# edlanglois/relearn

Hardware: AMD Instinct MI355X
Metric: env-steps/sec (whole node), 64k-env CartPole TRPO (higher is better)
Workload: dtype f32; 1 GPU; CartPole(VisibleStepLimit 500) MLP-TRPO, 65536 envs total, T=128, policy 5-128-2, critic 5-128-1, CG 10, <=15 backtracks, 80 Adam critic steps per period; n_envs_total=65536, n_envs_per_gpu=65536, horizon=128, hidden=128, critic_steps=80, update_chains=policy and critic chains side by side on two streams, pipeline=none, parallelism=env-sharded x1 + no collective (one rank)

## Files before the change

### include/relearn_hip.h

```cpp
#ifndef RELEARN_HIP_H
#define RELEARN_HIP_H

#include <stddef.h>
#include <stdint.h>

#ifdef __cplusplus
extern "C" {
#endif

#define RL_ABI_VERSION 6

typedef enum {
  RL_OK = 0,
  RL_ERR_INVALID_ARGUMENT = 1,
  RL_ERR_HIP = 2,
  RL_ERR_NO_DEVICE = 3,
  RL_ERR_BUILD_AGENT = 4,
  RL_ERR_BUILD_ENV = 5,
  RL_ERR_BUFFER_FULL = 6,
  RL_ERR_PACKING = 7,
  RL_ERR_COMM = 8,
  RL_ERR_OPT_NAN = 9,
  RL_ERR_UNSUPPORTED = 10
} rl_status;
// ... 117 lines not shown
enum { RL_CELL_GRU = 0, RL_CELL_LSTM = 1 };
int32_t rl_rnn_mlp_create(rl_engine *engine, int32_t cell, uint32_t in_dim, uint32_t hidden_size, uint32_t num_layers,
                          uint32_t mlp_hidden, uint32_t out_dim, rl_mlp **out);
int32_t rl_rnn_mlp_create_config(rl_engine *engine, int32_t cell, uint32_t in_dim, uint32_t hidden_size,
                                 uint32_t num_layers, int32_t bias, uint32_t mlp_hidden, uint32_t out_dim, rl_mlp **out);

typedef enum {
  RL_TRAJ_OBS = 0,
  RL_TRAJ_ACTION = 1,
  RL_TRAJ_REWARD = 2,
  RL_TRAJ_FLAG = 3,
  RL_TRAJ_TERM_OBS = 4,
  RL_TRAJ_VALUES = 5,
  RL_TRAJ_ADVANTAGES = 6,
  RL_TRAJ_RETURNS = 7,
  RL_TRAJ_TARGETS = 8
} rl_traj_field;

int32_t rl_traj_create(rl_engine *engine, uint64_t n_lanes, uint64_t horizon, uint32_t obs_dim, rl_traj **out);
int32_t rl_traj_destroy(rl_traj *traj);
int32_t rl_traj_field_bytes(const rl_traj *traj, int32_t field, uint64_t *bytes);
int32_t rl_traj_read(rl_traj *traj, int32_t field, void *host, uint64_t bytes);
int32_t rl_traj_write(rl_traj *traj, int32_t field, const void *host, uint64_t bytes);

int32_t rl_rollout(rl_env *env, const rl_mlp *policy, rl_traj *traj);

int32_t rl_gae(rl_traj *traj, const rl_mlp *critic, float gamma, float lambda);
int32_t rl_seq_forward(rl_mlp *module, rl_traj *traj, float *out, float *succ_out);

typedef struct {
  uint64_t iterations;
// ... 169 lines not shown
```

### relearn_amd/__init__.py

```python
import atexit
import ctypes as C
import math
import os
import subprocess
import sys
import weakref

import numpy as np

_HERE = os.path.dirname(os.path.abspath(__file__))
LIB_PATH = os.environ.get("RELEARN_LIB", os.path.join(_HERE, "librelearn_hip.so"))
CSRC = os.path.join(_HERE, "csrc")

OK = 0
ERR_INVALID_ARGUMENT, ERR_HIP, ERR_NO_DEVICE, ERR_BUILD_AGENT, ERR_BUILD_ENV = 1, 2, 3, 4, 5
ERR_BUFFER_FULL, ERR_PACKING, ERR_COMM, ERR_OPT_NAN, ERR_UNSUPPORTED = 6, 7, 8, 9, 10
SUCC_CONTINUE, SUCC_TERMINATE, SUCC_INTERRUPT = 0, 1, 2
OPT_OK, OPT_LOSS_NOT_IMPROVING, OPT_CONSTRAINT_VIOLATED, OPT_NAN_LOSS, OPT_NAN_CONSTRAINT = range(5)
ENV_CARTPOLE, ENV_CHAIN, ENV_MEMORY, ENV_BANDIT = 0, 1, 2, 3
LIMIT_NONE, LIMIT_LATENT, LIMIT_VISIBLE = 0, 1, 2
(TRAJ_OBS, TRAJ_ACTION, TRAJ_REWARD, TRAJ_FLAG, TRAJ_TERM_OBS, TRAJ_VALUES, TRAJ_ADVANTAGES,
 TRAJ_RETURNS, TRAJ_TARGETS) = range(9)
VALUE_TARGET_REWARD_TO_GO, VALUE_TARGET_ONE_STEP_TD = 0, 1
KERNEL_CLASSES = ["env_step", "rollout", "values", "gae", "policy_pass", "backward", "reduce", "small",
                  "critic_fwd", "allreduce", "critic_fused", "policy_fused", "policy_fvp"]

ABI_SYMBOLS = [
    "rl_abi_version", "rl_debug_stream_words", "rl_device_count", "rl_engine_create", "rl_engine_destroy", "rl_engine_sync",
    "rl_last_error", "rl_engine_info", "rl_engine_set_kernel_variant", "rl_timer_begin", "rl_timer_end", "rl_profile_enable", "rl_profile_read",
    "rl_comm_available", "rl_comm_library_paths", "rl_comm_unique_id", "rl_comm_init", "rl_comm_destroy", "rl_comm_init_host",
    "rl_comm_ipc_handle", "rl_comm_init_ipc", "rl_comm_selftest",
    "rl_cartpole_params_default", "rl_env_create", "rl_env_destroy", "rl_env_dims", "rl_env_reset",
    "rl_env_observe", "rl_env_step", "rl_env_upload_actions", "rl_env_step_resident", "rl_env_get_state",
    "rl_env_set_state",
    "rl_mlp_create", "rl_mlp_create_layers", "rl_mlp_create_config", "rl_mlp_destroy", "rl_mlp_num_params", "rl_mlp_init", "rl_mlp_init_with", "rl_params_get", "rl_params_set",
    "rl_mlp_forward", "rl_gru_mlp_create", "rl_lstm_mlp_create", "rl_rnn_mlp_create", "rl_rnn_mlp_create_config", "rl_rnn_mlp_init_with", "rl_seq_forward",
    "rl_traj_create", "rl_traj_destroy", "rl_traj_field_bytes", "rl_traj_read", "rl_traj_write",
# ... 521 lines not shown
    def forward(self, rows):
        rows, rp = _ptr(rows, np.float32)
        out = np.zeros((rows.shape[0], self.out_dim), dtype=np.float32)
        _check(lib().rl_mlp_forward(self.h, rp, C.c_uint64(rows.shape[0]), out.ctypes.data_as(C.c_void_p)),
               self.eng.h)
        return out


GruMlp.close = Mlp.close
GruMlp.init = Mlp.init
GruMlp.get_params = Mlp.get_params
GruMlp.set_params = Mlp.set_params

_TRAJ_DTYPES = {TRAJ_OBS: np.float32, TRAJ_ACTION: np.uint8, TRAJ_REWARD: np.float32, TRAJ_FLAG: np.uint8,
                TRAJ_TERM_OBS: np.float32, TRAJ_VALUES: np.float32, TRAJ_ADVANTAGES: np.float32,
                TRAJ_RETURNS: np.float32, TRAJ_TARGETS: np.float32}


class Trajectory(_Handle):
    def __init__(self, engine, n_lanes, horizon, obs_dim):
        self.eng = engine
        self.h = C.c_void_p()
        _check(lib().rl_traj_create(engine.h, C.c_uint64(n_lanes), C.c_uint64(horizon), C.c_uint32(obs_dim),
                                    C.byref(self.h)), engine.h)
        _register(self)
        self.n, self.T, self.D = n_lanes, horizon, obs_dim

    def close(self):
        if self.h:
            lib().rl_traj_destroy(self.h)
            self.h = C.c_void_p()

    def shape(self, field):
        n, T, D = self.n, self.T, self.D
        return {TRAJ_OBS: (D, T + 1, n), TRAJ_ACTION: (T, n), TRAJ_REWARD: (T, n), TRAJ_FLAG: (T, n),
                TRAJ_TERM_OBS: (D, T, n), TRAJ_VALUES: (T + 1, n), TRAJ_ADVANTAGES: (T, n),
                TRAJ_RETURNS: (T, n), TRAJ_TARGETS: (T, n)}[field]

    def read(self, field):
        out = np.zeros(self.shape(field), dtype=_TRAJ_DTYPES[field])
        _check(lib().rl_traj_read(self.h, C.c_int32(field), out.ctypes.data_as(C.c_void_p),
                                  C.c_uint64(out.nbytes)), self.eng.h)
        return out

    def write(self, field, arr):
        arr, ap = _ptr(arr, _TRAJ_DTYPES[field])
        assert arr.shape == self.shape(field), (arr.shape, self.shape(field))
        _check(lib().rl_traj_write(self.h, C.c_int32(field), ap, C.c_uint64(arr.nbytes)), self.eng.h)

    def read_all(self):
        return dict(obs=self.read(TRAJ_OBS), action=self.read(TRAJ_ACTION), reward=self.read(TRAJ_REWARD),
                    flag=self.read(TRAJ_FLAG), term_obs=self.read(TRAJ_TERM_OBS))
# ... 427 lines not shown
```

### relearn_amd/csrc/abi.hip

```cpp
#include <dlfcn.h>

#include <atomic>
#include <condition_variable>
#include <map>
#include <mutex>

#include "abi_internal.hpp"

thread_local std::string g_last_error_no_engine;

ProfScope::ProfScope(rl_engine *eng, int c) : e(eng), cls(c) {
  if (!e->profiling) return;
  auto get = [&]() {
    hipEvent_t ev;
    if (!e->prof_event_pool.empty()) {
      ev = e->prof_event_pool.back();
      e->prof_event_pool.pop_back();
    } else if (hipEventCreate(&ev) != hipSuccess) {
      ev = nullptr;
    }
    return ev;
  };
  a = get();
  b = get();
// ... 1273 lines not shown
  uint64_t n = t->d.n, T = t->d.T, D = t->d.D;
  switch (field) {
    case RL_TRAJ_OBS: *ptr = t->d.obs; *bytes = D * (T + 1) * n * 4; break;
    case RL_TRAJ_ACTION: *ptr = t->d.action; *bytes = T * n; break;
    case RL_TRAJ_REWARD: *ptr = t->d.reward; *bytes = T * n * 4; break;
    case RL_TRAJ_FLAG: *ptr = t->d.flag; *bytes = T * n; break;
    case RL_TRAJ_TERM_OBS: *ptr = t->d.term_obs; *bytes = D * T * n * 4; break;
    case RL_TRAJ_VALUES: *ptr = t->d.values; *bytes = (T + 1) * n * 4; break;
    case RL_TRAJ_ADVANTAGES: *ptr = t->d.adv; *bytes = T * n * 4; break;
    case RL_TRAJ_RETURNS: *ptr = t->d.rtg; *bytes = T * n * 4; break;
    case RL_TRAJ_TARGETS:
      RL_REQUIRE(t->last_targets != nullptr, "no value targets yet: they are written by rl_values_opt_update");
      *ptr = const_cast<float *>(t->last_targets);
      *bytes = T * n * 4;
      break;
    default: throw RlError(RL_ERR_INVALID_ARGUMENT, "unknown trajectory field");
  }
}

void traj_plan(rl_traj *t, uint64_t B) {
  rl_engine *e = t->eng;
  t->B = B;
  uint64_t chunk = (B + 1023) / 1024;
  chunk = ((chunk + 7) / 8) * 8;
  if (chunk < 64) chunk = 64;
  t->bwd_chunk = (uint32_t)chunk;
  t->nbA = (uint32_t)((B + chunk - 1) / chunk);
  uint64_t nbB = (B + 255) / 256;
  if (nbB > 2048) nbB = 2048;
  t->nbB = (uint32_t)nbB;
// ... 31 lines not shown
  t->d.tgt = t->d.rtg;
  t->d.range = dalloc<uint32_t>(RL_RANGE_ALLOC_WORDS);
  RL_HIP_CHECK(hipMemsetAsync(t->d.range, 0, RL_RANGE_ALLOC_WORDS * sizeof(uint32_t), e->stream));
  {
    void *hp = nullptr;
    RL_HIP_CHECK(hipHostMalloc(&hp, 64, hipHostMallocMapped));
    static_cast<volatile uint32_t *>(hp)[RL_GUARD_POLICY] = 0u;
    static_cast<volatile uint32_t *>(hp)[RL_GUARD_CRITIC] = 0u;
    void *dp = nullptr;
    RL_HIP_CHECK(hipHostGetDevicePointer(&dp, hp, 0));
    t->h_range_err = static_cast<uint32_t *>(hp);
    t->d.range_err = static_cast<uint32_t *>(dp);
  }
  t->lp0 = dalloc<float>(2 * n * T);
  t->dz = dalloc<float>(2 * n * T);
  t->Pmax = 128 * 5 + 128 + 2 * 128 + 2;
  traj_plan(t.get(), n * T);
  uint32_t rows = t->nbA;
  if (t->nbV2 > rows) rows = t->nbV2;
  if (t->nbC > rows) rows = t->nbC;
  uint32_t rowsB = t->nbB > rows ? t->nbB : rows;
  if (resizable) {
    uint32_t cap = 8u * (uint32_t)e->prop.multiProcessorCount;
    if (cap < 2048) cap = 2048;
    rows = rowsB = cap;
  }
  t->slabA = dalloc<double>((size_t)rows * t->Pmax);
  t->slabB = dalloc<double>((size_t)rowsB * 4);
  t->cap_slabA = (uint64_t)rows * t->Pmax;
  t->cap_slabB = (uint64_t)rowsB * 4;
// ... 21 lines not shown
    RL_REQUIRE(e && out, "NULL argument");
    *out = nullptr;
    *out = traj_alloc(e, n_lanes, horizon, obs_dim, false);
  });
}

static void seq_free(rl_traj *t);

int32_t rl_traj_destroy(rl_traj *t) {
  if (!t) return RL_OK;
  (void)hipSetDevice(t->eng->device);
  (void)hipStreamSynchronize(t->eng->main_stream);
  (void)hipStreamSynchronize(t->eng->aux_stream);
  if (t->eng->pending.traj == t) t->eng->pending.active = false;
  void *ptrs[] = {t->d.obs, t->d.action, t->d.reward, t->d.flag, t->d.term_obs, t->d.values, t->d.adv, t->d.rtg,
                  t->lp0, t->dz, t->slabA, t->slabB, t->vec, t->cg_x, t->cg_r, t->cg_p, t->prev_params, t->descent,
                  t->losses, t->trpo, t->td, t->aux_slabA, t->aux_slabB, t->aux_vec, t->d.range};
  for (void *p : ptrs) dfree(p);
  if (t->h_range_err) (void)hipHostFree(t->h_range_err);
  seq_free(t);
  gen_free(t);
  rl_engine *eng = t->eng;
  delete t;
  engine_release_child(eng);
  return RL_OK;
}

int32_t rl_traj_field_bytes(const rl_traj *t, int32_t field, uint64_t *bytes) {
  return guarded(t ? t->eng : nullptr, [&] {
    RL_REQUIRE(t && bytes, "NULL argument");
    void *p;
// ... 5 lines not shown
  return guarded(t ? t->eng : nullptr, [&] {
    RL_REQUIRE(t && host, "NULL argument");
    void *p;
    uint64_t need;
    traj_field(t, field, &p, &need);
    RL_REQUIRE(bytes == need, "byte count mismatch for trajectory field");
    d2h(t->eng, host, p, bytes);
  });
}

int32_t rl_traj_write(rl_traj *t, int32_t field, const void *host, uint64_t bytes) {
  return guarded(t ? t->eng : nullptr, [&] {
    RL_REQUIRE(t && host, "NULL argument");
    void *p;
    uint64_t need;
    traj_field(t, field, &p, &need);
    RL_REQUIRE(bytes == need, "byte count mismatch for trajectory field");
    h2d(t->eng, p, host, bytes);
    if (field == RL_TRAJ_OBS) t->range_valid = t->range_reset = false;
    t->rtg_scan_valid = false;
  });
}

void traj_ensure_pvec(rl_traj *t, uint64_t P) {
  if (t->Pmax >= P) return;
  for (float **p : {&t->vec, &t->cg_x, &t->cg_r, &t->cg_p, &t->prev_params, &t->descent}) {
    dfree(*p);
    *p = nullptr;
  }
  t->Pmax = (uint32_t)P;
// ... 117 lines not shown
```

### relearn_amd/csrc/abi_update.hip

```cpp
#include "abi_internal.hpp"

extern "C" {

static void seq_gradient_to_flat_order(const rl_mlp *mod, rl_traj *traj) {
  if (mod->exec == nullptr) return;
  launch_seq_unpad(mod, traj->vec, mod->x_tmp);
  RL_HIP_CHECK(hipMemcpyAsync(traj->vec, mod->x_tmp, mod->P * sizeof(float), hipMemcpyDeviceToDevice, traj->eng->stream));
}

static float *seq_record(rl_traj *traj, const rl_mlp *mod) {
  return mod->lane_kernels() ? traj->seq.stack.rec : traj->seq.act;
}

static void seq_policy_pass(rl_mlp *policy, rl_traj *traj, int mode, bool backward, float lo, float hi) {
  SeqScope sc(traj, policy);
  seq_ensure(traj, sc.x, true);
  uint32_t P = (uint32_t)policy->P;
  launch_gru_seq_forward(traj, sc.x, traj->seq.out, nullptr, backward ? seq_record(traj, sc.x) : nullptr);
  launch_seq_policy_dlogits(traj, mode, b_total(traj), lo, hi);
  if (backward) {
    launch_gru_backward(traj, sc.x);
    seq_gradient_to_flat_order(policy, traj);
  }
  launch_reduce(traj, P, false, true, 0, traj->nbB);
// ... 43 lines not shown
    c->iterations = 10;
    c->max_backtracks = 15;
    c->backtrack_ratio = 0.8;
    c->hpv_reg_coeff = 1e-5;
    c->max_policy_step_kl = 0.01;
    c->accept_violation = 0;
  });
}

static void check_policy(const rl_mlp *policy, const rl_traj *traj) {
  RL_REQUIRE(policy && traj, "NULL argument");
  RL_REQUIRE(policy->eng == traj->eng, "handles belong to different engines");
  RL_REQUIRE(policy->in_dim == traj->d.D && policy->out_dim == 2, "policy shape does not match the trajectory");
}

static void run_policy_gradient(rl_mlp *policy, rl_traj *traj) {
  if (rl_module_is_recurrent(policy->kind)) return seq_policy_pass(policy, traj, PASS_INIT, true, 0.0f, 0.0f);
  uint32_t P = (uint32_t)policy->P;
  if (traj->eng->kernel_variant != 1 && launch_policy_v2(traj, policy, PASS_INIT, nullptr, b_total(traj), nullptr)) {
    launch_reduce(traj, P, true, true, traj->last_rows, traj->last_rows);
  } else {
    launch_policy_pass(traj, policy, PASS_INIT, nullptr, b_total(traj), nullptr);
    launch_mlp_backward(traj, policy, nullptr);
    launch_reduce(traj, P, true, true, traj->nbA, traj->nbB);
  }
  rl_allreduce_sum_f32(traj->eng, traj->vec, P + 4);
}

static void run_policy_eval(rl_mlp *policy, rl_traj *traj, const int32_t *d_skip) {
  if (rl_module_is_recurrent(policy->kind)) return seq_policy_eval(policy, traj, d_skip);
  uint32_t P = (uint32_t)policy->P;
  if (traj->eng->kernel_variant != 1 && launch_policy_v2(traj, policy, PASS_EVAL, nullptr, b_total(traj), d_skip)) {
    launch_reduce(traj, P, false, true, traj->last_rows, traj->last_rows);
  } else {
// ... 19 lines not shown
static inline void trpo_candidate(rl_mlp *policy, rl_traj *traj, const rl_trpo_config *cfg, uint64_t i, double ratio) {
  launch_ls_set_params(traj, policy, ratio);
  run_policy_eval(policy, traj, &traj->trpo->ls_accepted);
  launch_ls_check(traj, (uint32_t)policy->P, b_total(traj), (int)i, ratio, cfg->max_policy_step_kl);
}

struct TrpoProgress {
  uint64_t next = 0;
  double ratio = 1.0;
};

static TrpoProgress trpo_update_head(rl_mlp *policy, rl_traj *traj, const rl_trpo_config *cfg) {
  uint32_t P = (uint32_t)policy->P;
  uint64_t Bt = b_total(traj);
  float reg = (float)cfg->hpv_reg_coeff;
  run_policy_gradient(policy, traj);
  launch_trpo_begin(traj, policy, Bt);
  for (uint64_t it = 0; it < cfg->iterations; ++it) {
    run_policy_fvp(policy, traj, traj->cg_p, &traj->trpo->cg_done);
    launch_cg_step(traj, P, reg, 1e-10f);
  }
  launch_cg_finish(traj, P);
  run_policy_fvp(policy, traj, traj->cg_x, nullptr);
  launch_step_size(traj, policy, reg, cfg->max_policy_step_kl);
  TrpoProgress pr;
  for (; pr.next < cfg->max_backtracks && pr.next < 2; ++pr.next) {
    if (pr.next > 0) pr.ratio *= cfg->backtrack_ratio;
    trpo_candidate(policy, traj, cfg, pr.next, pr.ratio);
  }
  return pr;
}
// ... 562 lines not shown
```

### relearn_amd/csrc/bf16_tile.hpp

```cpp
#pragma once
#include <hip/hip_runtime.h>

#include <cstdint>

namespace bt {

typedef float f32x16 __attribute__((ext_vector_type(16)));
typedef float f32x2 __attribute__((ext_vector_type(2)));
typedef __bf16 bf16x8 __attribute__((ext_vector_type(8)));
typedef __bf16 bf16x2 __attribute__((ext_vector_type(2)));

constexpr int NT = 4;
constexpr uint32_t SHARE_OLD = 5, SHARE_YOUNG = 3;
constexpr int COLS = 19;
constexpr int UROW = 36;

__device__ __forceinline__ void wave_lds_fence() {
  __builtin_amdgcn_fence(__ATOMIC_RELEASE, "wavefront");
  __builtin_amdgcn_wave_barrier();
  __builtin_amdgcn_fence(__ATOMIC_ACQUIRE, "wavefront");
}

__device__ __forceinline__ uint32_t pack_bf16(float lo, float hi) {
  const f32x2 x = {lo, hi};
// ... 34 lines not shown
constexpr int YROW = 36;
__device__ __forceinline__ float row_sum16v(const float *row) {
  const float4 *v = reinterpret_cast<const float4 *>(row);
  const float4 q0 = v[0], q1 = v[1], q2 = v[2], q3 = v[3];
  const float a0 = ((q0.x + q1.x) + q2.x) + q3.x, a1 = ((q0.y + q1.y) + q2.y) + q3.y;
  const float a2 = ((q0.z + q1.z) + q2.z) + q3.z, a3 = ((q0.w + q1.w) + q2.w) + q3.w;
  return (a0 + a1) + (a2 + a3);
}

typedef __amdgpu_buffer_rsrc_t rsrc_t;
__device__ __forceinline__ rsrc_t make_rsrc(const void *p, uint32_t bytes) {
  return __builtin_amdgcn_make_buffer_rsrc(const_cast<void *>(p), 0, (int)bytes, 0x00020000);
}
__device__ __forceinline__ float buf_f32(rsrc_t r, uint32_t lane_off, uint32_t tile_off) {
  return __builtin_bit_cast(float, __builtin_amdgcn_raw_buffer_load_b32(r, (int)lane_off, (int)tile_off, 0));
}
__device__ __forceinline__ uint32_t buf_u8(rsrc_t r, uint32_t lane_off, uint32_t tile_off) {
  return (uint32_t)__builtin_amdgcn_raw_buffer_load_b8(r, (int)lane_off, (int)tile_off, 0);
}

union Frag {
  bf16x8 v;
  uint32_t u[4];
  uint64_t q[2];
  uint4 x;
};

__device__ __forceinline__ void weight_frags(float wa, float wb, float w4, float bias, int hf, Frag (&f)[3]) {
  uint32_t a0, a1, a2, c0, c1, c2, e0, e1, e2, g0, g1, g2;
  split3(wa, a0, a1, a2);
// ... 191 lines not shown
}

__device__ __forceinline__ uint32_t mask_pair(float lo, float hi, float after) {
  uint32_t r;
  asm("v_cvt_pk_bf16_f32 %0, %1, %2 clamp" : "=v"(r) : "v"(lo), "v"(hi), "v"(after));
  return r;
}
__device__ __forceinline__ void mask_tile(const f32x16 &c, Frag (&ga)[2]) {
  const float first = __builtin_amdgcn_fmed3f(c[0], 0.0f, 1.0f);
#pragma unroll
  for (int s = 0; s < 2; ++s)
#pragma unroll
    for (int i = 0; i < 4; ++i)
      ga[s].u[i] = mask_pair(s + i == 0 ? first : c[8 * s + 2 * i], c[8 * s + 2 * i + 1], first);
}

constexpr int L2_KS = 8;
__device__ __forceinline__ constexpr int acc_row(int s, int h, int e) { return 16 * s + 8 * (e >> 2) + 4 * h + (e & 3); }
__device__ __forceinline__ void ident_frags(int lane, Frag (&id)[2]) {
  const int n = lane & 31, hh = lane >> 5;
#pragma unroll
  for (int s = 0; s < 2; ++s)
#pragma unroll
    for (int i = 0; i < 4; ++i)
      id[s].u[i] = pk(acc_row(s, hh, 2 * i) == n ? 0x3F80u : 0u, acc_row(s, hh, 2 * i + 1) == n ? 0x3F80u : 0u);
}
template <typename F>
__device__ __forceinline__ void l2_build(uint4 (*img)[64], int tid, int nthreads, F val) {
  for (int idx = tid; idx < L2_KS * 64; idx += nthreads) {
    const int ks = idx >> 6, ln = idx & 63, m = ln & 31, hh = ln >> 5;
// ... 142 lines not shown
```

### relearn_amd/csrc/engine.hpp

```cpp
#pragma once

#include <hip/hip_runtime.h>

#include <cstdint>
#include <cstdio>
#include <stdexcept>
#include <string>
#include <vector>

#include "../../include/relearn_hip.h"

struct RlError : std::runtime_error {
  int32_t code;
  RlError(int32_t c, const std::string &m) : std::runtime_error(m), code(c) {}
};

#define RL_HIP_CHECK(expr)                                                                          \
  do {                                                                                              \
    hipError_t _e = (expr);                                                                         \
    if (_e != hipSuccess)                                                                           \
      throw RlError(RL_ERR_HIP, std::string(#expr) + ": " + hipGetErrorString(_e) + " (" __FILE__ ":" + \
                                    std::to_string(__LINE__) + ")");                                \
  } while (0)

// ... 234 lines not shown
  rl_engine *eng;
  rl_mlp *mod;
  rl_adam_config cfg;
  float *d_m = nullptr, *d_v = nullptr;
  uint64_t *d_step = nullptr;
  uint64_t host_step = 0;
  uint64_t error_epoch = 0;
};

struct rl_traj {
  rl_engine *eng;
  TrajDev d;
  uint64_t B;
  float *lp0 = nullptr;
  float *dz = nullptr;
  double *slabA = nullptr;
  double *slabB = nullptr;
  float *vec = nullptr;
  float *cg_x = nullptr, *cg_r = nullptr, *cg_p = nullptr, *prev_params = nullptr, *descent = nullptr;
  float *td = nullptr;
  float *losses = nullptr;
  TrpoStateDev *trpo = nullptr;
  uint32_t nbA = 0, nbB = 0, nbV2 = 0, nbC = 0, Pmax = 0, max_losses = 0;
  uint32_t last_rows = 0;
  uint64_t cap_slabA = 0, cap_slabB = 0;
  double *aux_slabA = nullptr, *aux_slabB = nullptr;
  float *aux_vec = nullptr;
  uint64_t aux_cap_slabA = 0, aux_cap_slabB = 0;
  uint32_t aux_last_rows = 0;
  bool range_valid = false, range_fixed = false;
// ... 59 lines not shown
```

### relearn_amd/csrc/kernels.hpp

```cpp
#pragma once
#include <cstdlib>
#include <functional>
#define RL_SEQ_ACT_ARRAYS 9
#define RL_SEQ_DPRE_ARRAYS 6
#include "engine.hpp"

void launch_env_reset(rl_env *env);
void launch_env_observe(rl_env *env, float *d_obs);
void launch_env_step(rl_env *env);
void launch_rollout(rl_env *env, const rl_mlp *policy, rl_traj *traj);
void launch_values(rl_traj *traj, const rl_mlp *critic);
void launch_gae(rl_traj *traj, const rl_mlp *critic, float gamma, float lambda);
void launch_value_targets(rl_traj *traj, const rl_mlp *critic, float gamma);
void launch_mlp_forward_host_rows(rl_mlp *mlp, const float *d_in_soa, size_t rows, float *d_out_soa);
void launch_obs_range(rl_traj *traj);
inline void traj_ensure_range(rl_traj *traj) {
  if (traj->range_valid || traj->range_fixed) return;
  launch_obs_range(traj);
  traj->range_valid = true;
}

const uint32_t *wimg_ensure(const rl_mlp *m);
inline uint32_t *wimg_if_current(const rl_mlp *m) {
  return m->d_wimg != nullptr && m->wimg_epoch == m->eng->call_epoch ? m->d_wimg : nullptr;
// ... 8 lines not shown
void launch_reduce(rl_traj *traj, uint32_t P, bool useA, bool useB, uint32_t rowsA, uint32_t rowsB);

void launch_trpo_begin(rl_traj *traj, rl_mlp *policy, uint64_t B_total);
void launch_cg_step(rl_traj *traj, uint32_t P, float reg, float tol);
void launch_cg_finish(rl_traj *traj, uint32_t P);
void launch_step_size(rl_traj *traj, rl_mlp *policy, float reg, double max_kl);
void launch_ls_set_params(rl_traj *traj, rl_mlp *policy, double ratio);
void launch_ls_check(rl_traj *traj, uint32_t P, uint64_t B_total, int index, double ratio, double max_kl);
void launch_ls_finalize(rl_traj *traj, rl_mlp *policy, double max_kl, int accept_violation);
void launch_adam_step(rl_traj *traj, rl_adam *opt, int loss_slot, uint64_t B_total);
void launch_adam_step_vec(rl_adam *opt, const float *d_grad);
void launch_reduce_adam(rl_traj *traj, rl_adam *opt, uint32_t rowsA, uint32_t rowsB, int loss_slot, uint64_t B_total);

bool launch_critic_step_v2(rl_traj *traj, const rl_mlp *critic, uint64_t B_total);
bool launch_policy_v2(rl_traj *traj, const rl_mlp *policy, int mode, const float *d_tangent, uint64_t B_total,
                      const int32_t *d_skip_flag, float clip_lo = 0.0f, float clip_hi = 0.0f);

void launch_rollout_dqn(rl_env *env, const rl_mlp *qnet, const ReplayDev &rp, uint32_t T, uint64_t p_int,
                        int always_explore, uint8_t *d_flags, uint32_t *d_range = nullptr);
void launch_rollout_dqn_general(rl_env *env, const rl_mlp *qnet, rl_traj *ws, float *d_q, const ReplayDev &rp, uint32_t T,
                                uint64_t p_int, int always_explore, uint8_t *d_flags);
void launch_dqn_td_targets(rl_engine *eng, float *d_target, const uint8_t *d_flag, const float *d_q_next, uint32_t n,
                           float gamma);
struct AgentKey { uint32_t w[8]; };
void launch_dqn_sample(rl_engine *eng, hipStream_t stream, const ReplayDev &rp, const AgentKey &key, uint64_t *d_agent_pos,
                       uint32_t minibatch_steps, uint32_t max_eps, uint32_t *d_lane, uint32_t *d_start,
                       uint32_t *d_len, uint32_t *d_off, DqnCountsDev *d_counts, int sequential,
                       uint32_t n_batches = 1);
void launch_dqn_build_all(rl_engine *eng, const ReplayDev &rp, uint32_t n_batches, uint32_t widest_eps, uint32_t max_eps,
                          const uint32_t *d_lane, const uint32_t *d_start, const uint32_t *d_len, const uint32_t *d_off,
                          const DqnCountsDev *d_counts, float *d_obs, size_t obs_stride, uint8_t *d_action,
// ... 59 lines not shown
```

### relearn_amd/csrc/kernels_mfma.hip

```cpp
#include <type_traits>

#include "bf16_tile.hpp"
#include "device_fns.hpp"
#include "kernels.hpp"
#include "policy_fast.hpp"

constexpr int V2_WAVES = 8;

constexpr int PB_FLUSH = 16;

template <int MODE, int WAVES, bool FW_LDS = false>
__global__ void __launch_bounds__(WAVES * 64)
    k_policy_bf16(TrajDev tr, const float *__restrict__ params, const uint32_t *__restrict__ wimg,
                  const float *__restrict__ tangent, float *__restrict__ lp0, double *__restrict__ slabA,
                  double *__restrict__ slabB, float inv_B, uint32_t P, const int32_t *__restrict__ skip, float clip_lo,
                  float clip_hi, uint32_t share_old, uint32_t share_young) {
  using bt::Frag;
  constexpr int D = 5, H = 128, NT = bt::NT, A = 2;
  constexpr bool BWD = MODE != PASS_EVAL;
  constexpr bool JVP = MODE == PASS_JVP;
  constexpr int IW = 7;
  constexpr int PIMG_M = H * IW + 5;
  __shared__ __attribute__((aligned(16))) float Ysh[JVP ? 1 : WAVES][32][bt::YROW];
  __shared__ double Acc[WAVES][BWD ? PIMG_M : 4];
  __shared__ uint4 Fz[JVP ? bt::L2_KS : 1][64];
  __shared__ uint4 Fw[FW_LDS ? NT * 3 : 1][64];
  if (skip != nullptr && *skip != 0) return;

  const int lane = threadIdx.x & 63;
  const int wave = __builtin_amdgcn_readfirstlane((int)(threadIdx.x >> 6));
  const int n = lane & 31, hf = lane >> 5;
  const float *__restrict__ W1 = params, *__restrict__ b1 = W1 + H * D, *__restrict__ W2 = b1 + H,
                           *__restrict__ b2 = W2 + A * H;
  const size_t B = (size_t)tr.T * tr.n;
  const size_t plane = (size_t)(tr.T + 1) * tr.n;
  double *acc64 = Acc[wave];
  bool flushed = false;

  Frag fw[NT][3];
  float w2d[NT];
  float lvd[3] = {0.0f, 0.0f, 0.0f};
  float tb2d = 0.0f;
  const bool guard = blockIdx.x == 0 && wave == 0 && tr.range != nullptr;
  float gxmin = 0.0f, gxmax = 0.0f;
  if (guard) bt::range_bounds(tr.range, lane, gxmin, gxmax);
#pragma unroll
  for (int t = 0; t < NT; ++t) {
    bt::WRaw r;
    bt::wimg_load(wimg, t, lane, fw[t], r, 2);
    if (guard)
      bt::range_guard_img(r, hf, gxmin, gxmax, tr.range_err + bt::GUARD_POLICY, bt::range_veto(tr.range, bt::GUARD_POLICY));
    if (FW_LDS && wave == t) {
#pragma unroll
      for (int i = 0; i < 3; ++i) Fw[t * 3 + i][lane] = fw[t][i].x;
    }
    const float wd = r.w2[0] - r.w2[1];
    if (!JVP) {
      lvd[0] = __builtin_fmaf(wd, r.wa, lvd[0]);
      lvd[1] = __builtin_fmaf(wd, r.wb, lvd[1]);
      lvd[2] = __builtin_fmaf(wd, r.wc, lvd[2]);
    }
    w2d[t] = bt::FWD_UNSCALE * wd;
// ... 47 lines not shown
    return p0 + p1;
  };

  const uint32_t B32 = (uint32_t)B, plane32 = (uint32_t)plane;
  const uint32_t n_full = B32 / 32u, tail = B32 & 31u;
  if (WAVES != 8) share_old = share_young = 1u;
  const uint32_t per_wg = (WAVES / 2) * (share_old + share_young);
  const uint32_t my_share = wave < WAVES / 2 ? share_old : share_young;
  const uint32_t my_first = blockIdx.x * per_wg + (wave < WAVES / 2 ? (uint32_t)wave * share_old
                                                   : (WAVES / 2) * share_old + (uint32_t)(wave - WAVES / 2) * share_young);
  const uint32_t n_waves = gridDim.x * per_wg;
  const bt::rsrc_t obs_r = bt::make_rsrc(tr.obs, (uint32_t)D * plane32 * 4u), lp0_r = bt::make_rsrc(lp0, 2u * B32 * 4u);
  const bt::rsrc_t adv_r = bt::make_rsrc(tr.adv, B32 * 4u), act_r = bt::make_rsrc(tr.action, B32);
  const uint32_t off_a = ((uint32_t)(2 * hf) * plane32 + (uint32_t)n) * 4u, off_b = off_a + plane32 * 4u;
  const uint32_t off_c = (4u * plane32 + (uint32_t)n) * 4u, off_s = (uint32_t)n * 4u, off_s1 = off_s + B32 * 4u;
  int since_flush = 0;
  struct TileOp {
    float xa, xb, xc, l0, l1, adv;
    int act;
  };
  auto load_tile = [&](uint32_t g) {
    TileOp o;
    const uint32_t soff = g * 128u;
    o.xa = bt::buf_f32(obs_r, off_a, soff);
    o.xb = bt::buf_f32(obs_r, off_b, soff);
    o.xc = bt::buf_f32(obs_r, off_c, soff);
    o.l0 = o.l1 = o.adv = 0.0f;
    o.act = 0;
    if (MODE != PASS_INIT) {
      o.l0 = bt::buf_f32(lp0_r, off_s, soff);
      o.l1 = bt::buf_f32(lp0_r, off_s1, soff);
    }
    if (!JVP) {
      o.adv = bt::buf_f32(adv_r, off_s, soff);
      o.act = (int)bt::buf_u8(act_r, (uint32_t)n, g * 32u);
    }
    return o;
  };
  auto tile = [&](auto ragged, TileOp op_in, uint32_t g) {
    constexpr bool RAGGED = decltype(ragged)::value;
    struct {
      float xa, xb, xc, l0, l1, adv;
      int act;
      bool valid;
    } op;
    op.valid = RAGGED ? (uint32_t)n < tail : true;
    op.xa = op.valid ? op_in.xa : 0.0f;
    op.xb = op.valid ? op_in.xb : 0.0f;
    op.xc = op.valid ? op_in.xc : 0.0f;
    op.l0 = op.valid ? op_in.l0 : 0.0f;
    op.l1 = op.valid ? op_in.l1 : 0.0f;
    op.adv = op.valid ? op_in.adv : 0.0f;
    op.act = op.valid ? op_in.act : 0;
    const size_t sidx = (size_t)g * 32 + n;
    Frag fa[3];
    bt::input_frags(op.xa, op.xb, op.xc, op.valid, hf, fa);
    Frag ga[NT][2];
    float y0[16];
#pragma unroll
    for (int r = 0; r < 16; ++r) y0[r] = 0.0f;
    bt::f32x16 q = {0, 0, 0, 0, 0, 0, 0, 0, 0, 0, 0, 0, 0, 0, 0, 0};
    auto fwd = [&](int t) {
      if (FW_LDS) {
        Frag f[3];
#pragma unroll
        for (int i = 0; i < 3; ++i) f[i].x = Fw[t * 3 + i][lane];
        return bt::layer1(fa, f);
      }
      return bt::layer1(fa, fw[t]);
    };
    bt::f32x16 c = fwd(0);
#pragma unroll
    for (int t = 0; t < NT; ++t) {
      bt::f32x16 cn = c;
      if (t + 1 < NT) cn = fwd(t + 1);
      if (!JVP) {
#pragma unroll
        for (int r = 0; r < 16; ++r) y0[r] = __builtin_fmaf(__builtin_fabsf(c[r]), w2d[t], y0[r]);
      }
      if (BWD) bt::mask_tile(c, ga[t]);
      if (JVP) q = bt::masked_sum_tile(ga[t], idb, Fz, t, lane, q);
      c = cn;
    }
    float s0;
    if (JVP) {
      float p0, p1;
      bt::both_halves(bt::l2_dot(q, op.xa, op.xb, hf == 0 ? op.xc : 1.0f), p0, p1);
      s0 = p0 + p1;
    } else {
      float lin = lvd[0] * op.xa;
      lin = __builtin_fmaf(lvd[1], op.xb, lin);
      lin = __builtin_fmaf(lvd[2], hf == 0 ? op.xc : 1.0f, lin);
      s0 = 0.5f * lane_sum(y0, lin);
    }
    float dz0 = 0.0f, dz1 = 0.0f;
    if (JVP) {
      const float delta = s0 + tb2d;
// ... 48 lines not shown
        const SoftPair old = soft_pair(l00 - l01);
        float kl = rel0 * old.p[0];
        kl += rel1 * old.p[1];
        if (op.valid) {
          s0f = __builtin_fmaf(ratio, adv, s0f);
          s1f = s1f + kl;
        }
      }
    }
    if (BWD) {
      d0f = d0f + dz0;
      d1f = d1f + dz1;
      Frag ub[2];
      bt::piece_frags_mfma(0.5f * (dz0 - dz1), op.xa, op.xb, op.xc, hf, selb, ub);
      bt::backward(ga, ub, dm);
      if (++since_flush == PB_FLUSH) {
        since_flush = 0;
        bt::flush(dm, acc64, IW, n, hf, !flushed);
        flushed = true;
        fold();
      }
    } else if (++since_flush == PB_FLUSH) {
      since_flush = 0;
      fold();
    }
  };
  for (uint32_t vw = 0; vw < my_share; ++vw) {
   const uint32_t wave_id = my_first + vw;
   if (wave_id < n_full) {
    TileOp op_a = load_tile(wave_id), op_b = op_a;
// ... 77 lines not shown
    }
  }
  if (threadIdx.x < 4) {
    double v = 0.0;
    if (BWD) {
      if (!JVP && threadIdx.x < 2) v = tot(TAIL + 2 + threadIdx.x);
      if (MODE == PASS_INIT && threadIdx.x == 2) v = tot(TAIL + 4);
    } else if (threadIdx.x < 2) {
      v = tot(threadIdx.x);
    }
    slabB[(size_t)blockIdx.x * 4 + threadIdx.x] = v;
  }
}

bool launch_policy_v2(rl_traj *traj, const rl_mlp *policy, int mode, const float *d_tangent, uint64_t B_total,
                      const int32_t *d_skip, float clip_lo, float clip_hi) {
  if (policy->general) return launch_gen_mfma(traj, policy, mode, d_tangent, B_total, d_skip, clip_lo, clip_hi);
  if (traj->d.D != 5 || policy->hidden != 128 || policy->out_dim != 2) return false;
  if (mode == PASS_DQN) return false;
  if ((uint64_t)(traj->d.T + 1) * traj->d.n * 5 >= (1ull << 30)) return false;
  traj_ensure_range(traj);
  const uint32_t *wimg = wimg_ensure(policy);
  ProfScope ps(traj->eng, mode == PASS_JVP ? RL_K_POLICY_FVP : RL_K_POLICY_FUSED);
  float inv_B = 1.0f / (float)B_total;
  traj->last_rows = traj->nbV2;
  dim3 g(traj->nbV2), b(V2_WAVES * 64);
  hipStream_t s = traj->eng->stream;
  uint32_t P = (uint32_t)policy->P;
  TrajDev d = traj->d;
  if (!traj->guard_next_policy) d.range = nullptr;
  traj->guard_next_policy = false;
#define BLAUNCH(MM)                                                                                                  \
  hipLaunchKernelGGL((k_policy_bf16<MM, V2_WAVES>), g, b, 0, s, d, policy->d_params, wimg, d_tangent, traj->lp0,       \
                     traj->slabA, traj->slabB, inv_B, P, d_skip, clip_lo, clip_hi, bt::SHARE_OLD, bt::SHARE_YOUNG)
  if (mode == PASS_INIT) BLAUNCH(PASS_INIT);
  else if (mode == PASS_JVP) BLAUNCH(PASS_JVP);
  else if (mode == PASS_PPO) BLAUNCH(PASS_PPO);
  else {
    constexpr int EVAL_WAVES = 16;
    hipLaunchKernelGGL((k_policy_bf16<PASS_EVAL, EVAL_WAVES, true>), g, dim3(EVAL_WAVES * 64), 0, s, d,
                       policy->d_params, wimg, d_tangent, traj->lp0, traj->slabA, traj->slabB, inv_B, P, d_skip, clip_lo,
                       clip_hi, 1u, 1u);
  }
#undef BLAUNCH
  return true;
}
```

### relearn_amd/csrc/kernels_update.hip

```cpp
#include "bf16_tile.hpp"
#include "comm_ipc.hpp"
#include "device_fns.hpp"
#include "kernels.hpp"
#include "policy_terms.hpp"

#include <cfloat>
#include <cmath>

static inline uint32_t cdiv(size_t a, size_t b) { return (uint32_t)((a + b - 1) / b); }

template <int D, int MODE>
__global__ void __launch_bounds__(256) k_policy_pass(TrajDev tr, const float *__restrict__ params,
                                                     const float *__restrict__ tangent, int H,
                                                     float *__restrict__ lp0, float *__restrict__ dz,
                                                     double *__restrict__ slabB, float inv_B,
                                                     const int32_t *__restrict__ skip, float clip_lo,
                                                     float clip_hi) {
  constexpr int A = 2;
  __shared__ double red[256];
  if (skip != nullptr && *skip != 0) return;
  const size_t B = (size_t)tr.T * tr.n;
  const size_t plane = (size_t)(tr.T + 1) * tr.n;
  double s0 = 0.0, s1 = 0.0, s2 = 0.0;
  for (size_t b = (size_t)blockIdx.x * 256 + threadIdx.x; b < B; b += (size_t)gridDim.x * 256) {
// ... 690 lines not shown
}

void launch_cg_finish(rl_traj *traj, uint32_t P) {
  ProfScope ps(traj->eng, RL_K_SMALL);
  hipLaunchKernelGGL(k_cg_finish, dim3(1), dim3(SB), 0, traj->eng->stream, traj->cg_x, P);
}

void launch_step_size(rl_traj *traj, rl_mlp *policy, float reg, double max_kl) {
  ProfScope ps(traj->eng, RL_K_SMALL);
  hipLaunchKernelGGL(k_step_size, dim3(1), dim3(SB), 0, traj->eng->stream, traj->vec, (uint32_t)policy->P, reg,
                     max_kl, traj->cg_x, traj->descent, policy->d_params, traj->prev_params, traj->trpo);
}

void launch_ls_set_params(rl_traj *traj, rl_mlp *policy, double ratio) {
  ProfScope ps(traj->eng, RL_K_SMALL);
  hipLaunchKernelGGL(k_ls_set_params, dim3(1), dim3(SB), 0, traj->eng->stream, policy->d_params, traj->prev_params,
                     traj->descent, (uint32_t)policy->P, (float)ratio, traj->trpo, comm_err_word(traj->eng),
                     wimg_if_current(policy), (int)policy->out_dim);
}

const uint32_t *wimg_ensure(const rl_mlp *m) {
  rl_engine *e = m->eng;
  if (m->d_wimg == nullptr) {
    RL_HIP_CHECK(hipSetDevice(e->device));
    void *p = nullptr;
    RL_HIP_CHECK(hipMalloc(&p, (size_t)bt::WIMG_WORDS * sizeof(uint32_t)));
    m->d_wimg = static_cast<uint32_t *>(p);
    m->wimg_epoch = 0;
  }
  if (m->wimg_epoch != e->call_epoch) {
// ... 95 lines not shown
```

Measured before the change: 495.8 million env-steps/s.

## Record ReLU masks in the gradient pass and reuse them in CG FVP passes

The initial policy-gradient pass now writes a compact bitmask of hidden-layer ReLU activations per sample into a new trajectory buffer. The JVP passes inside the conjugate-gradient loop read those masks instead of recomputing the first-layer forward, skipping the weight-image loads and the input MFMA. The record is invalidated when line-search parameters change, and it adds a 16-byte per-sample read in place of the forward compute.

```diff
diff --git a/include/relearn_hip.h b/include/relearn_hip.h
--- a/include/relearn_hip.h
+++ b/include/relearn_hip.h
@@ -155,7 +155,8 @@
   RL_TRAJ_VALUES = 5,
   RL_TRAJ_ADVANTAGES = 6,
   RL_TRAJ_RETURNS = 7,
-  RL_TRAJ_TARGETS = 8
+  RL_TRAJ_TARGETS = 8,
+  RL_TRAJ_POLICY_MASKS = 9
 } rl_traj_field;
 
 int32_t rl_traj_create(rl_engine *engine, uint64_t n_lanes, uint64_t horizon, uint32_t obs_dim, rl_traj **out);
diff --git a/relearn_amd/__init__.py b/relearn_amd/__init__.py
--- a/relearn_amd/__init__.py
+++ b/relearn_amd/__init__.py
@@ -20,7 +20,7 @@
 ENV_CARTPOLE, ENV_CHAIN, ENV_MEMORY, ENV_BANDIT = 0, 1, 2, 3
 LIMIT_NONE, LIMIT_LATENT, LIMIT_VISIBLE = 0, 1, 2
 (TRAJ_OBS, TRAJ_ACTION, TRAJ_REWARD, TRAJ_FLAG, TRAJ_TERM_OBS, TRAJ_VALUES, TRAJ_ADVANTAGES,
- TRAJ_RETURNS, TRAJ_TARGETS) = range(9)
+ TRAJ_RETURNS, TRAJ_TARGETS, TRAJ_POLICY_MASKS) = range(10)
 VALUE_TARGET_REWARD_TO_GO, VALUE_TARGET_ONE_STEP_TD = 0, 1
 KERNEL_CLASSES = ["env_step", "rollout", "values", "gae", "policy_pass", "backward", "reduce", "small",
                   "critic_fwd", "allreduce", "critic_fused", "policy_fused", "policy_fvp"]
@@ -572,7 +572,7 @@
 
 _TRAJ_DTYPES = {TRAJ_OBS: np.float32, TRAJ_ACTION: np.uint8, TRAJ_REWARD: np.float32, TRAJ_FLAG: np.uint8,
                 TRAJ_TERM_OBS: np.float32, TRAJ_VALUES: np.float32, TRAJ_ADVANTAGES: np.float32,
-                TRAJ_RETURNS: np.float32, TRAJ_TARGETS: np.float32}
+                TRAJ_RETURNS: np.float32, TRAJ_TARGETS: np.float32, TRAJ_POLICY_MASKS: np.uint32}
 
 
 class Trajectory(_Handle):
@@ -593,7 +593,7 @@
         n, T, D = self.n, self.T, self.D
         return {TRAJ_OBS: (D, T + 1, n), TRAJ_ACTION: (T, n), TRAJ_REWARD: (T, n), TRAJ_FLAG: (T, n),
                 TRAJ_TERM_OBS: (D, T, n), TRAJ_VALUES: (T + 1, n), TRAJ_ADVANTAGES: (T, n),
-                TRAJ_RETURNS: (T, n), TRAJ_TARGETS: (T, n)}[field]
+                TRAJ_RETURNS: (T, n), TRAJ_TARGETS: (T, n), TRAJ_POLICY_MASKS: ((T * n + 31) // 32, 32, 4)}[field]
 
     def read(self, field):
         out = np.zeros(self.shape(field), dtype=_TRAJ_DTYPES[field])
diff --git a/relearn_amd/csrc/abi.hip b/relearn_amd/csrc/abi.hip
--- a/relearn_amd/csrc/abi.hip
+++ b/relearn_amd/csrc/abi.hip
@@ -1311,6 +1311,7 @@
       *ptr = const_cast<float *>(t->last_targets);
       *bytes = T * n * 4;
       break;
+    case RL_TRAJ_POLICY_MASKS: *ptr = t->mrec; *bytes = (T * n + 31) / 32 * 512; break;
     default: throw RlError(RL_ERR_INVALID_ARGUMENT, "unknown trajectory field");
   }
 }
@@ -1372,6 +1373,7 @@
   }
   t->lp0 = dalloc<float>(2 * n * T);
   t->dz = dalloc<float>(2 * n * T);
+  t->mrec = dalloc<uint32_t>((n * T + 31) / 32 * 128);
   t->Pmax = 128 * 5 + 128 + 2 * 128 + 2;
   traj_plan(t.get(), n * T);
   uint32_t rows = t->nbA;
@@ -1423,7 +1425,7 @@
   (void)hipStreamSynchronize(t->eng->aux_stream);
   if (t->eng->pending.traj == t) t->eng->pending.active = false;
   void *ptrs[] = {t->d.obs, t->d.action, t->d.reward, t->d.flag, t->d.term_obs, t->d.values, t->d.adv, t->d.rtg,
-                  t->lp0, t->dz, t->slabA, t->slabB, t->vec, t->cg_x, t->cg_r, t->cg_p, t->prev_params, t->descent,
+                  t->lp0, t->dz, t->mrec, t->slabA, t->slabB, t->vec, t->cg_x, t->cg_r, t->cg_p, t->prev_params, t->descent,
                   t->losses, t->trpo, t->td, t->aux_slabA, t->aux_slabB, t->aux_vec, t->d.range};
   for (void *p : ptrs) dfree(p);
   if (t->h_range_err) (void)hipHostFree(t->h_range_err);
@@ -1459,6 +1461,7 @@
     RL_REQUIRE(t && host, "NULL argument");
     void *p;
     uint64_t need;
+    RL_REQUIRE(field != RL_TRAJ_POLICY_MASKS, "the policy mask record is written by the library only");
     traj_field(t, field, &p, &need);
     RL_REQUIRE(bytes == need, "byte count mismatch for trajectory field");
     h2d(t->eng, p, host, bytes);
diff --git a/relearn_amd/csrc/abi_update.hip b/relearn_amd/csrc/abi_update.hip
--- a/relearn_amd/csrc/abi_update.hip
+++ b/relearn_amd/csrc/abi_update.hip
@@ -81,10 +81,11 @@
   RL_REQUIRE(policy->in_dim == traj->d.D && policy->out_dim == 2, "policy shape does not match the trajectory");
 }
 
-static void run_policy_gradient(rl_mlp *policy, rl_traj *traj) {
+static void run_policy_gradient(rl_mlp *policy, rl_traj *traj, bool mask_record = false) {
   if (rl_module_is_recurrent(policy->kind)) return seq_policy_pass(policy, traj, PASS_INIT, true, 0.0f, 0.0f);
   uint32_t P = (uint32_t)policy->P;
-  if (traj->eng->kernel_variant != 1 && launch_policy_v2(traj, policy, PASS_INIT, nullptr, b_total(traj), nullptr)) {
+  if (traj->eng->kernel_variant != 1 &&
+      launch_policy_v2(traj, policy, PASS_INIT, nullptr, b_total(traj), nullptr, 0.0f, 0.0f, mask_record)) {
     launch_reduce(traj, P, true, true, traj->last_rows, traj->last_rows);
   } else {
     launch_policy_pass(traj, policy, PASS_INIT, nullptr, b_total(traj), nullptr);
@@ -134,7 +135,7 @@
   uint32_t P = (uint32_t)policy->P;
   uint64_t Bt = b_total(traj);
   float reg = (float)cfg->hpv_reg_coeff;
-  run_policy_gradient(policy, traj);
+  run_policy_gradient(policy, traj, true);
   launch_trpo_begin(traj, policy, Bt);
   for (uint64_t it = 0; it < cfg->iterations; ++it) {
     run_policy_fvp(policy, traj, traj->cg_p, &traj->trpo->cg_done);
diff --git a/relearn_amd/csrc/bf16_tile.hpp b/relearn_amd/csrc/bf16_tile.hpp
--- a/relearn_amd/csrc/bf16_tile.hpp
+++ b/relearn_amd/csrc/bf16_tile.hpp
@@ -72,6 +72,9 @@
 }
 __device__ __forceinline__ float buf_f32(rsrc_t r, uint32_t lane_off, uint32_t tile_off) {
   return __builtin_bit_cast(float, __builtin_amdgcn_raw_buffer_load_b32(r, (int)lane_off, (int)tile_off, 0));
+}
+__device__ __forceinline__ uint4 buf_u128(rsrc_t r, uint32_t lane_off, uint32_t tile_off) {
+  return __builtin_bit_cast(uint4, __builtin_amdgcn_raw_buffer_load_b128(r, (int)lane_off, (int)tile_off, 0));
 }
 __device__ __forceinline__ uint32_t buf_u8(rsrc_t r, uint32_t lane_off, uint32_t tile_off) {
   return (uint32_t)__builtin_amdgcn_raw_buffer_load_b8(r, (int)lane_off, (int)tile_off, 0);
@@ -293,6 +296,27 @@
     for (int i = 0; i < 4; ++i)
       ga[s].u[i] = mask_pair(s + i == 0 ? first : c[8 * s + 2 * i], c[8 * s + 2 * i + 1], first);
 }
+__device__ __forceinline__ uint32_t mask_bits(const Frag (&ga)[2], int hf) {
+  uint32_t w = 0u;
+#pragma unroll
+  for (int s = 0; s < 2; ++s)
+#pragma unroll
+    for (int i = 0; i < 4; ++i) {
+      const int p = 4 * s + i;
+      w |= (ga[s].u[i] >> (7 - p)) & (0x10001u << p);
+    }
+  return w << (8 * hf);
+}
+__device__ __forceinline__ void unmask_tile(uint32_t word, int hf, Frag (&ga)[2]) {
+  const uint32_t w = word >> (8 * hf);
+#pragma unroll
+  for (int s = 0; s < 2; ++s)
+#pragma unroll
+    for (int i = 0; i < 4; ++i) {
+      const int p = 4 * s + i;
+      ga[s].u[i] = (w & (0x10001u << p)) * (0x3F80u >> p);
+    }
+}
 
 constexpr int L2_KS = 8;
 __device__ __forceinline__ constexpr int acc_row(int s, int h, int e) { return 16 * s + 8 * (e >> 2) + 4 * h + (e & 3); }
diff --git a/relearn_amd/csrc/engine.hpp b/relearn_amd/csrc/engine.hpp
--- a/relearn_amd/csrc/engine.hpp
+++ b/relearn_amd/csrc/engine.hpp
@@ -272,6 +272,9 @@
   uint64_t B;
   float *lp0 = nullptr;
   float *dz = nullptr;
+  uint32_t *mrec = nullptr;
+  uint64_t mrec_epoch = 0;
+  const struct rl_mlp *mrec_policy = nullptr;
   double *slabA = nullptr;
   double *slabB = nullptr;
   float *vec = nullptr;
diff --git a/relearn_amd/csrc/kernels.hpp b/relearn_amd/csrc/kernels.hpp
--- a/relearn_amd/csrc/kernels.hpp
+++ b/relearn_amd/csrc/kernels.hpp
@@ -46,7 +46,11 @@
 
 bool launch_critic_step_v2(rl_traj *traj, const rl_mlp *critic, uint64_t B_total);
 bool launch_policy_v2(rl_traj *traj, const rl_mlp *policy, int mode, const float *d_tangent, uint64_t B_total,
-                      const int32_t *d_skip_flag, float clip_lo = 0.0f, float clip_hi = 0.0f);
+                      const int32_t *d_skip_flag, float clip_lo = 0.0f, float clip_hi = 0.0f, bool mask_record = false);
+inline bool traj_mrec_current(const rl_traj *traj, const rl_mlp *policy) {
+  return traj->mrec != nullptr && traj->mrec_policy == policy && traj->mrec_epoch == traj->eng->call_epoch;
+}
+inline void traj_mrec_invalidate(rl_traj *traj) { traj->mrec_epoch = 0; }
 
 void launch_rollout_dqn(rl_env *env, const rl_mlp *qnet, const ReplayDev &rp, uint32_t T, uint64_t p_int,
                         int always_explore, uint8_t *d_flags, uint32_t *d_range = nullptr);
diff --git a/relearn_amd/csrc/kernels_mfma.hip b/relearn_amd/csrc/kernels_mfma.hip
--- a/relearn_amd/csrc/kernels_mfma.hip
+++ b/relearn_amd/csrc/kernels_mfma.hip
@@ -9,16 +9,18 @@
 
 constexpr int PB_FLUSH = 16;
 
-template <int MODE, int WAVES, bool FW_LDS = false>
+template <int MODE, int WAVES, bool FW_LDS = false, bool MREC = false>
 __global__ void __launch_bounds__(WAVES * 64)
     k_policy_bf16(TrajDev tr, const float *__restrict__ params, const uint32_t *__restrict__ wimg,
                   const float *__restrict__ tangent, float *__restrict__ lp0, double *__restrict__ slabA,
                   double *__restrict__ slabB, float inv_B, uint32_t P, const int32_t *__restrict__ skip, float clip_lo,
-                  float clip_hi, uint32_t share_old, uint32_t share_young) {
+                  float clip_hi, uint32_t share_old, uint32_t share_young, uint32_t *__restrict__ mrec) {
   using bt::Frag;
   constexpr int D = 5, H = 128, NT = bt::NT, A = 2;
   constexpr bool BWD = MODE != PASS_EVAL;
   constexpr bool JVP = MODE == PASS_JVP;
+  static_assert(!MREC || MODE == PASS_INIT || MODE == PASS_JVP, "the mask record: written by PASS_INIT, read by PASS_JVP");
+  constexpr bool REC_W = MREC && MODE == PASS_INIT, REC_R = MREC && JVP;
   constexpr int IW = 7;
   constexpr int PIMG_M = H * IW + 5;
   __shared__ __attribute__((aligned(16))) float Ysh[JVP ? 1 : WAVES][32][bt::YROW];
@@ -41,11 +43,12 @@
   float w2d[NT];
   float lvd[3] = {0.0f, 0.0f, 0.0f};
   float tb2d = 0.0f;
-  const bool guard = blockIdx.x == 0 && wave == 0 && tr.range != nullptr;
+  const bool guard = !REC_R && blockIdx.x == 0 && wave == 0 && tr.range != nullptr;
   float gxmin = 0.0f, gxmax = 0.0f;
   if (guard) bt::range_bounds(tr.range, lane, gxmin, gxmax);
 #pragma unroll
   for (int t = 0; t < NT; ++t) {
+    if (REC_R) break;
     bt::WRaw r;
     bt::wimg_load(wimg, t, lane, fw[t], r, 2);
     if (guard)
@@ -123,10 +126,12 @@
   const bt::rsrc_t adv_r = bt::make_rsrc(tr.adv, B32 * 4u), act_r = bt::make_rsrc(tr.action, B32);
   const uint32_t off_a = ((uint32_t)(2 * hf) * plane32 + (uint32_t)n) * 4u, off_b = off_a + plane32 * 4u;
   const uint32_t off_c = (4u * plane32 + (uint32_t)n) * 4u, off_s = (uint32_t)n * 4u, off_s1 = off_s + B32 * 4u;
+  const bt::rsrc_t mrec_r = bt::make_rsrc(mrec, REC_R ? ((B32 + 31u) / 32u) * 512u : 0u);
   int since_flush = 0;
   struct TileOp {
     float xa, xb, xc, l0, l1, adv;
     int act;
+    uint4 mr;
   };
   auto load_tile = [&](uint32_t g) {
     TileOp o;
@@ -144,6 +149,8 @@
       o.adv = bt::buf_f32(adv_r, off_s, soff);
       o.act = (int)bt::buf_u8(act_r, (uint32_t)n, g * 32u);
     }
+    o.mr = make_uint4(0u, 0u, 0u, 0u);
+    if (REC_R) o.mr = bt::buf_u128(mrec_r, (uint32_t)n * 16u, g * 512u);
     return o;
   };
   auto tile = [&](auto ragged, TileOp op_in, uint32_t g) {
@@ -163,12 +170,20 @@
     op.act = op.valid ? op_in.act : 0;
     const size_t sidx = (size_t)g * 32 + n;
     Frag fa[3];
-    bt::input_frags(op.xa, op.xb, op.xc, op.valid, hf, fa);
+    if (!REC_R) bt::input_frags(op.xa, op.xb, op.xc, op.valid, hf, fa);
     Frag ga[NT][2];
     float y0[16];
 #pragma unroll
     for (int r = 0; r < 16; ++r) y0[r] = 0.0f;
     bt::f32x16 q = {0, 0, 0, 0, 0, 0, 0, 0, 0, 0, 0, 0, 0, 0, 0, 0};
+    if (REC_R) {
+      const uint32_t mw[NT] = {op_in.mr.x, op_in.mr.y, op_in.mr.z, op_in.mr.w};
+#pragma unroll
+      for (int t = 0; t < NT; ++t) {
+        bt::unmask_tile(mw[t], hf, ga[t]);
+        q = bt::masked_sum_tile(ga[t], idb, Fz, t, lane, q);
+      }
+    } else {
     auto fwd = [&](int t) {
       if (FW_LDS) {
         Frag f[3];
@@ -190,6 +205,7 @@
       if (BWD) bt::mask_tile(c, ga[t]);
       if (JVP) q = bt::masked_sum_tile(ga[t], idb, Fz, t, lane, q);
       c = cn;
+    }
     }
     float s0;
     if (JVP) {
@@ -268,6 +284,16 @@
       Frag ub[2];
       bt::piece_frags_mfma(0.5f * (dz0 - dz1), op.xa, op.xb, op.xc, hf, selb, ub);
       bt::backward(ga, ub, dm);
+      if (REC_W) {
+        uint32_t mw[NT];
+#pragma unroll
+        for (int t = 0; t < NT; ++t) {
+          float lo, hi;
+          bt::both_halves(__builtin_bit_cast(float, bt::mask_bits(ga[t], hf)), lo, hi);
+          mw[t] = __builtin_bit_cast(uint32_t, lo) | __builtin_bit_cast(uint32_t, hi);
+        }
+        if (hf == 0) reinterpret_cast<uint4 *>(mrec)[(size_t)g * 32 + n] = make_uint4(mw[0], mw[1], mw[2], mw[3]);
+      }
       if (++since_flush == PB_FLUSH) {
         since_flush = 0;
         bt::flush(dm, acc64, IW, n, hf, !flushed);
@@ -375,7 +401,7 @@
 }
 
 bool launch_policy_v2(rl_traj *traj, const rl_mlp *policy, int mode, const float *d_tangent, uint64_t B_total,
-                      const int32_t *d_skip, float clip_lo, float clip_hi) {
+                      const int32_t *d_skip, float clip_lo, float clip_hi, bool mask_record) {
   if (policy->general) return launch_gen_mfma(traj, policy, mode, d_tangent, B_total, d_skip, clip_lo, clip_hi);
   if (traj->d.D != 5 || policy->hidden != 128 || policy->out_dim != 2) return false;
   if (mode == PASS_DQN) return false;
@@ -391,17 +417,27 @@
   TrajDev d = traj->d;
   if (!traj->guard_next_policy) d.range = nullptr;
   traj->guard_next_policy = false;
-#define BLAUNCH(MM)                                                                                                  \
-  hipLaunchKernelGGL((k_policy_bf16<MM, V2_WAVES>), g, b, 0, s, d, policy->d_params, wimg, d_tangent, traj->lp0,       \
-                     traj->slabA, traj->slabB, inv_B, P, d_skip, clip_lo, clip_hi, bt::SHARE_OLD, bt::SHARE_YOUNG)
-  if (mode == PASS_INIT) BLAUNCH(PASS_INIT);
-  else if (mode == PASS_JVP) BLAUNCH(PASS_JVP);
-  else if (mode == PASS_PPO) BLAUNCH(PASS_PPO);
-  else {
+#define BLAUNCH(MM, REC)                                                                                             \
+  hipLaunchKernelGGL((k_policy_bf16<MM, V2_WAVES, false, REC>), g, b, 0, s, d, policy->d_params, wimg, d_tangent,     \
+                     traj->lp0, traj->slabA, traj->slabB, inv_B, P, d_skip, clip_lo, clip_hi, bt::SHARE_OLD,          \
+                     bt::SHARE_YOUNG, traj->mrec)
+  if (mode == PASS_INIT && mask_record) {
+    BLAUNCH(PASS_INIT, true);
+    traj->mrec_epoch = traj->eng->call_epoch;
+    traj->mrec_policy = policy;
+  } else if (mode == PASS_INIT) {
+    BLAUNCH(PASS_INIT, false);
+  } else if (mode == PASS_JVP && traj_mrec_current(traj, policy)) {
+    BLAUNCH(PASS_JVP, true);
+  } else if (mode == PASS_JVP) {
+    BLAUNCH(PASS_JVP, false);
+  } else if (mode == PASS_PPO) {
+    BLAUNCH(PASS_PPO, false);
+  } else {
     constexpr int EVAL_WAVES = 16;
     hipLaunchKernelGGL((k_policy_bf16<PASS_EVAL, EVAL_WAVES, true>), g, dim3(EVAL_WAVES * 64), 0, s, d,
                        policy->d_params, wimg, d_tangent, traj->lp0, traj->slabA, traj->slabB, inv_B, P, d_skip, clip_lo,
-                       clip_hi, 1u, 1u);
+                       clip_hi, 1u, 1u, nullptr);
   }
 #undef BLAUNCH
   return true;
diff --git a/relearn_amd/csrc/kernels_update.hip b/relearn_amd/csrc/kernels_update.hip
--- a/relearn_amd/csrc/kernels_update.hip
+++ b/relearn_amd/csrc/kernels_update.hip
@@ -728,6 +728,7 @@
 
 void launch_ls_set_params(rl_traj *traj, rl_mlp *policy, double ratio) {
   ProfScope ps(traj->eng, RL_K_SMALL);
+  traj_mrec_invalidate(traj);
   hipLaunchKernelGGL(k_ls_set_params, dim3(1), dim3(SB), 0, traj->eng->stream, policy->d_params, traj->prev_params,
                      traj->descent, (uint32_t)policy->P, (float)ratio, traj->trpo, comm_err_word(traj->eng),
                      wimg_if_current(policy), (int)policy->out_dim);
```

Result: no change. 495.1 million env-steps/s, median of 4 (-0.1%).
